# AwesomePeiweiPan/Droid-SLAM_Reserch

Measured on AMD Instinct MI355X. Metric: BA update iters/sec (2000-edge equivalents; 256 keyframes, 48x64), higher is better.
Workload: dtype f32; 1 GPU; 256-keyframe / 2000-edge global BA, 48x64, t0=1, lm=1e-5 ep=1e-2 (BASELINE configs[2]); edges_total=2000, solve=fp64 dense Cholesky on device, chol_failed=False

## Files before the change

droid-slam_reserch_amd/csrc/api.hip:

```cpp
#include <hip/hip_runtime.h>
#include <stdarg.h>
#include <stdio.h>

#include <map>
#include <mutex>

#include "../../include/droid_backends_hip.h"
#include "../../include/droid_test_hooks_hip.h"
#include "../../include/droid_heads_hip.h"
#include "../../include/droid_motion_encode_hip.h"
#include "../../include/droid_update_hip.h"
#include "ba_internal.hpp"
#include "graph.hpp"
#include "launchers.hpp"

using namespace droid;

static thread_local char g_err[512] = "";

static std::map<const void*, int*> g_mirror;
static std::mutex g_mirror_mu;
struct HintState { int* ptr; int tag; };
static std::map<const void*, HintState> g_hint;
static int g_hint_tag = 0;
// ... 241 lines not shown
static void enqueue_build(const BaView& v, const float* poses, const float* disps, const float* intrinsics,
                          const float* disps_sens, const float* targets, const float* weights, const float* eta,
                          const int64_t* ii, const int64_t* jj, bool motion_only, hipStream_t s, Between between) {
  const BaLaunchPlan plan = ba_launch_plan(v);
  for (int stage = 0; stage < 3; stage++) {
    launch_build_stage(v, plan, poses, disps, intrinsics, disps_sens, targets, weights, eta, ii, jj, motion_only, stage, s);
    between();
  }
}
template <class Between>
static void enqueue_solve_update(const BaView& v, float* poses, float* disps, const float* intrinsics, const float* weights,
                                 const int64_t* ii, const int64_t* jj, float lm, float ep, bool motion_only, float* dx_out,
                                 float* dz_out, int* status_mirror, hipStream_t s, Between between) {
  const CholSystem c(v);
  if (v.E <= 0) launch_chol_preset(c, s);
  const bool single = launch_chol_factor(c, (double)lm, (double)ep, s);
  between();
  launch_chol_backsolve(c, single, s);
  between();
  launch_update(v, poses, disps, intrinsics, weights, ii, jj, v.xsol, dx_out, dz_out, motion_only, s, status_mirror);
  between();
}

static int ba_build_impl(const float* poses, const float* disps, const float* intrinsics,
                         const float* disps_sens, const float* targets, const float* weights,
                         const float* eta, const int64_t* ii, const int64_t* jj, const BaDims& d, void* workspace,
                         size_t workspace_bytes, void* stream, int packed) {
  BaView v;
  int rc = ba_view(v, workspace, workspace_bytes, d);
  if (rc) return rc;
  v.packed = packed;
  hints_of(v, workspace, false);
  if (!poses || !disps || !intrinsics) return fail(DROID_E_ARG, "ba: null %s", "state pointer");
// ... 91 lines not shown
}

int droid_ba_solve_update_overlap(float* poses, float* disps, const float* intrinsics, const float* weights,
                                  const int64_t* ii, const int64_t* jj, int E, int nbuf, int H, int W, int M,
                                  int t0, int t1, int epoch, int motion_only, float* dx_out, float* dz_out,
                                  void* workspace, size_t workspace_bytes, void* stream) {
  BaView v;
  int rc = ba_view(v, workspace, workspace_bytes, BaDims{E, nbuf, H, W, M, t0, t1, motion_only});
  if (!rc) rc = solve_update_check(poses, disps, intrinsics, weights, ii, jj, E, motion_only);
  if (rc) return rc;
  if (E <= 0 || epoch <= 0) return fail(DROID_E_ARG, "ba_solve_update_overlap: needs %s", "edges (the build presets the solver scratch) and epoch > 0");
  hipStream_t s = (hipStream_t)stream;
  const CholSystem c(v);
  if (!launch_chol_factor_overlap(c, v.ov_ready, epoch, s))
    return fail(DROID_E_ARG, "ba_solve_update_overlap: %s", "the single-launch solver is not available for this system (unpack and call droid_ba_solve_update)");
  launch_chol_backsolve(c, true, s);
  launch_update(v, poses, disps, intrinsics, weights, ii, jj, v.xsol, dx_out, dz_out, motion_only != 0, s,
                mirror_of(workspace));
  return check_hip("ba_solve_update_overlap");
}

int droid_ba_solve_update(float* poses, float* disps, const float* intrinsics, const float* weights,
                          const int64_t* ii, const int64_t* jj, int E, int nbuf, int H, int W, int M,
                          int t0, int t1, float lm, float ep, int motion_only, float* dx_out,
                          float* dz_out, void* workspace, size_t workspace_bytes, void* stream) {
  BaView v;
  int rc = ba_view(v, workspace, workspace_bytes, BaDims{E, nbuf, H, W, M, t0, t1, motion_only});
  if (!rc) rc = solve_update_check(poses, disps, intrinsics, weights, ii, jj, E, motion_only);
  if (rc) return rc;
  enqueue_solve_update(v, poses, disps, intrinsics, weights, ii, jj, lm, ep, motion_only != 0, dx_out, dz_out,
                       mirror_of(workspace), (hipStream_t)stream, [] {});
// ... 555 lines not shown
```

droid-slam_reserch_amd/csrc/ba_internal.hpp:

```cpp
#pragma once
#include <hip/hip_runtime.h>
#include <stddef.h>
#include <stdint.h>

namespace droid {

constexpr int LIN_THREADS = 256;
constexpr int LIN_PPT = 2;
constexpr int LIN_CP = LIN_THREADS * LIN_PPT;
constexpr int LIN_WAVES = LIN_THREADS / 64;
constexpr int CHOL_NB = 64;
__host__ __device__ inline int chol_ld(int n) { return (n + 1 + 15) & ~15; }
__host__ __device__ inline size_t chol_flag_words(int n) { return 2 * ((size_t)(n + 1 + CHOL_NB - 1) / CHOL_NB) + 8; }
__host__ __device__ inline int chol_tile_index(int nrb, int bi, int bj) { return bj * nrb - bj * (bj - 1) / 2 + (bi - bj); }
__host__ __device__ inline size_t chol_tiles(int n) {
  const int nb = (n + CHOL_NB - 1) / CHOL_NB, nrb = (n + 1 + CHOL_NB - 1) / CHOL_NB;
  return (size_t)chol_tile_index(nrb, nb, nb);
}
__host__ __device__ inline size_t chol_mbuf_offset(int n) { return ((size_t)(n + CHOL_NB - 1) / CHOL_NB) * CHOL_NB * CHOL_NB; }
__host__ __device__ inline size_t chol_lfin_offset(int n) { return 2 * chol_mbuf_offset(n); }
__host__ __device__ inline size_t chol_ldiag_doubles(int n) { return chol_lfin_offset(n) + chol_tiles(n) * CHOL_NB * CHOL_NB; }
__host__ __device__ inline int chol_bs_pairs_grid(int nb) { return (nb + 1) / 2; }
__host__ __device__ inline int chol_bs_pairs_owner(int col) { return col / 2; }
__host__ __device__ inline int chol_bs_pairs_first(int wg) { return 2 * wg; }

__host__ __device__ inline size_t pk_colbase(int n, int J) {
  return (size_t)CHOL_NB * ((size_t)J * (size_t)(n + 1) - (size_t)CHOL_NB * (size_t)J * (size_t)(J - 1) / 2);
}
// ... 188 lines not shown
};

void launch_wave_reduce32_test(const float* in, float* out, hipStream_t s);
void launch_lin_test(const BaView& v, const float* poses, const float* disps, const float* intr, const float* sens,
                     const float* targets, const float* weights, const float* eta, const int64_t* ii, const int64_t* jj,
                     bool motion_only, bool ragged, hipStream_t s);
void launch_prep(const BaView& v, const int64_t* ii, const int64_t* jj, hipStream_t s);
void launch_unpack_system(const BaView& v, hipStream_t s);
void launch_build_stage(const BaView& v, const BaLaunchPlan& plan, const float* poses, const float* disps,
                        const float* intr, const float* sens, const float* targets, const float* weights,
                        const float* eta, const int64_t* ii, const int64_t* jj, bool motion_only,
                        int stage, hipStream_t s);
void launch_update(const BaView& v, float* poses, float* disps, const float* intr, const float* weights,
                   const int64_t* ii, const int64_t* jj, const double* x, float* dx_out, float* dz_out,
                   bool motion_only, hipStream_t s, int* status_mirror = nullptr);
void launch_chol_preset(const CholSystem& c, hipStream_t s);
bool launch_chol_factor(const CholSystem& c, double lm, double ep, hipStream_t s);
void launch_chol_backsolve(const CholSystem& c, bool factor_single, hipStream_t s);
void launch_chol_solve(const CholSystem& c, double lm, double ep, hipStream_t s, bool preset_done);

void launch_unpack_cols(const BaView& v, int J0, int J1, double lm, double ep, int epoch, hipStream_t s);
bool launch_chol_factor_overlap(const CholSystem& c, const int* ready, int epoch, hipStream_t s);
bool chol_overlap_available(int n);

}
```

droid-slam_reserch_amd/csrc/chol.hip:

```cpp
#include <hip/hip_runtime.h>
#include <mutex>

#include <cstdint>
#include <cstdlib>

#include "ba_internal.hpp"
#include "launchers.hpp"

namespace droid {

constexpr int NB = CHOL_NB;

#ifdef CHOL_STAMPS
__device__ unsigned long long g_chol_stamps[64 * 16];
__device__ unsigned long long g_bs_stamps[64 * 8];
__shared__ unsigned long long g_chol_lstamps[16];
extern "C" int droid_debug_chol_stamps(unsigned long long* out) {
  return (int)hipMemcpyFromSymbol(out, HIP_SYMBOL(g_chol_stamps), sizeof(unsigned long long) * 64 * 16);
}
extern "C" int droid_debug_bs_stamps(unsigned long long* out) {
  return (int)hipMemcpyFromSymbol(out, HIP_SYMBOL(g_bs_stamps), sizeof(unsigned long long) * 64 * 8);
}
#define STEP_STAMP(slot)                                                                                      \
  do { if (threadIdx.x == 0 && panel && (blockIdx.x < 2))                                                      \
// ... 1 lines not shown
#define LDS_STAMP(slot)                                                                                       \
  do { if (threadIdx.x == 0 && panel && (bi - kp < 2)) {                                                       \
    g_chol_lstamps[slot] = wall_clock64();                                                                    \
    if ((slot) == 2) { g_chol_lstamps[14] = 0; g_chol_lstamps[15] = 0; g_chol_lstamps[9] = 0; }               \
    if ((slot) == 8)                                                                                          \
      for (int ss = 0; ss < 16; ss++)                                                                         \
        if (ss < 11 || ss > 13) g_chol_stamps[((k + 1) & 31) * 32 + (bi - kp) * 16 + ss] = g_chol_lstamps[ss]; \
  } } while (0)
#define TILE_STAMP(slot) do { if (PERSIST) LDS_STAMP(slot); else STEP_STAMP(slot); } while (0)
#define GEMM_STAMP_AT(slot) do { if (ASSIGN && threadIdx.x == 0 && g_chol_lstamps[slot] == 0) g_chol_lstamps[slot] = wall_clock64(); } while (0)
#define GEMM_STAMP_ENTERED() GEMM_STAMP_AT(9)
#define GEMM_STAMP_OPERANDS() do { asm volatile("s_waitcnt vmcnt(0) lgkmcnt(0)" ::: "memory"); GEMM_STAMP_AT(14); } while (0)
#define GEMM_STAMP_DONE(acc) do { asm volatile("s_nop 15\n s_nop 15" : "+v"(acc)); GEMM_STAMP_AT(15); } while (0)
#define WAIT_STAMP(slot) do { if (t == 0 && panel && (bi - kp < 2)) g_chol_stamps[(kp & 31) * 32 + (bi - kp) * 16 + (slot)] = wall_clock64(); } while (0)
#define BS_STAMP(slot) do { if (threadIdx.x == 0 && blockIdx.x < 64) g_bs_stamps[blockIdx.x * 8 + (slot)] = wall_clock64(); } while (0)
#else
#define TILE_STAMP(slot) do { } while (0)
#define GEMM_STAMP_ENTERED() do { } while (0)
#define GEMM_STAMP_OPERANDS() do { } while (0)
#define GEMM_STAMP_DONE(acc) do { } while (0)
#define WAIT_STAMP(slot) do { } while (0)
#define BS_STAMP(slot) do { } while (0)
#endif
#ifdef OV_DEBUG
__device__ unsigned long long g_ov_dbg[64];
extern "C" int droid_debug_overlap_stamps(unsigned long long* out) {
  return (int)hipMemcpyFromSymbol(out, HIP_SYMBOL(g_ov_dbg), sizeof(unsigned long long) * 64);
}
#define OV_STAMP_ENTERED() do { if (blockIdx.x == 0 && threadIdx.x == 0) g_ov_dbg[63] = wall_clock64(); } while (0)
#define OV_STAMP_DIAG(bi, bj, k) do { if (threadIdx.x == 0 && (bi) == (bj) && (bj) == (k) + 1 && (bj) < 62) g_ov_dbg[bj] = wall_clock64(); } while (0)
#else
// ... 68 lines not shown
}

template <bool COH = false>
__device__ __forceinline__ void store_tile64(gbl_f64* __restrict__ S, const lds_f64* __restrict__ src,
                                             int ld, int r0, int c0, int row_begin, int row_end,
                                             int ncols, bool lower) {
  const int t = threadIdx.x & 255;
  if (COH) {
#pragma unroll
    for (int it = 0; it < 8; it++) {
      const int idx2 = it * 256 + t;
      const int i = idx2 >> 5, j = (idx2 & 31) * 2;
      if (r0 + i >= row_begin && r0 + i < row_end && j < ncols) {
        gbl_f64* p = &S[(size_t)(r0 + i) * ld + c0 + j];
        const f64x2 v = *(const lds_f64x2*)&src[i * LDP + j];
        if (j + 1 < ncols) asm volatile("global_store_dwordx4 %0, %1, off sc1" ::"v"(p), "v"(v) : "memory");
        else gstore<true>(p, v[0]);
      }
    }
    return;
  }
#pragma unroll
  for (int it = 0; it < 16; it++) {
    const int idx = it * 256 + t;
    const int i = idx >> 6, j = idx & 63;
    if (r0 + i >= row_begin && r0 + i < row_end && j < ncols && (!lower || j <= i))
      S[(size_t)(r0 + i) * ld + c0 + j] = src[i * LDP + j];
  }
}

__device__ __forceinline__ double readlane_f64(double v, int lane) {
// ... 52 lines not shown
  a[J] *= y;
  w[J] *= y;
  asm volatile("s_nop 1" : "+v"(a[J]));
#pragma unroll
  for (int c = J + 1; c < 16; c++) {
    switch (c) {
#define DROID_CASE(CC) case CC: if (CC > J) { fmac_bcast<J, CC>(a[CC], a[J], a[J]); fmac_bcast<J, CC>(w[CC], a[J], w[J]); } break;
      DROID_CASE(1) DROID_CASE(2) DROID_CASE(3) DROID_CASE(4) DROID_CASE(5) DROID_CASE(6) DROID_CASE(7) DROID_CASE(8)
      DROID_CASE(9) DROID_CASE(10) DROID_CASE(11) DROID_CASE(12) DROID_CASE(13) DROID_CASE(14) DROID_CASE(15)
#undef DROID_CASE
      default: break;
    }
  }
}

__device__ __forceinline__ void wave_potrf16(lds_f64* Lb, lds_f64* Wl, const lds_f64* Idn, int* fail, bool report) {
  const int lane = threadIdx.x & 63, row = lane & 15;
  __builtin_amdgcn_s_setprio(3);
  double a[16], w[16];
#pragma unroll
  for (int c = 0; c < 16; c++) {
    a[c] = Lb[row * LDP + c];
    w[c] = Idn[row * WLP + c];
  }
  double ylast = 0.0;
  potrf16_pivot<0>(a, w, ylast);   potrf16_pivot<1>(a, w, ylast);   potrf16_pivot<2>(a, w, ylast);
  potrf16_pivot<3>(a, w, ylast);   potrf16_pivot<4>(a, w, ylast);   potrf16_pivot<5>(a, w, ylast);
  potrf16_pivot<6>(a, w, ylast);   potrf16_pivot<7>(a, w, ylast);   potrf16_pivot<8>(a, w, ylast);
  potrf16_pivot<9>(a, w, ylast);   potrf16_pivot<10>(a, w, ylast);  potrf16_pivot<11>(a, w, ylast);
  potrf16_pivot<12>(a, w, ylast);  potrf16_pivot<13>(a, w, ylast);  potrf16_pivot<14>(a, w, ylast);
  potrf16_pivot<15>(a, w, ylast);
// ... 119 lines not shown
    if (++spins > CFP_SPIN_LIMIT || ((spins & 255) == 0 && cfp_load(abortf) == 1)) {
      cfp_report_stall(fail, abortf);
      break;
    }
    __builtin_amdgcn_s_sleep(1);
  }
#pragma unroll
  for (int it = 0; it < 2; it++) {
    const int u = it * 256 + t;
    const int i = u >> 3, j = 16 * sp + (u & 7) * 2;
    if (!ok[it]) v[it] = (f64x2){0.0, 0.0};
    *(lds_f64x2*)(&dst[i * LDP + j]) = v[it];
  }
}

__shared__ double g_cholB0[NB * LDP];
__shared__ double g_cholB1[NB * LDP];
__shared__ double g_cholB2[NB * LDP];
__shared__ double g_cholBT[NB * LDP];
__shared__ double g_cholWl[4 * WLB];
__shared__ double g_cholIdn[WLB];

__device__ __forceinline__ void chol_strip_out(gbl_f64* __restrict__ S, int ld, gbl_f64* __restrict__ slot,
                                                         const lds_f64* __restrict__ BT, int r0, int c0, int wk, int nrows,
                                                         int p, int* done_flag, int done_value) {
  const int lane = threadIdx.x & 63;
  const int rb = max(r0, c0 + wk) - r0, re = min(r0 + NB, nrows) - r0;
  const int i0 = lane >> 3, j = 16 * p + (lane & 7) * 2;
  auto uniform = [](const gbl_f64* q) {
    const unsigned long long a = (unsigned long long)q;
    const unsigned lo = __builtin_amdgcn_readfirstlane((unsigned)a), hi = __builtin_amdgcn_readfirstlane((unsigned)(a >> 32));
    return (const gbl_f64*)(((unsigned long long)hi << 32) | lo);
  };
  const gbl_f64* sbase = uniform(S + (size_t)r0 * ld + c0);
  const gbl_f64* sslot = uniform(slot);
  unsigned off_slot = (unsigned)((i0 * NB + j) * 8), off_mat = (unsigned)((i0 * ld + j) * 8);
// ... 20 lines not shown
    off_mat += step_mat;
  }
  if (done_flag != nullptr) {
    asm volatile("s_waitcnt vmcnt(0)" ::: "memory");
    if (lane == 0) cfp_store(done_flag, done_value);
  }
}

template <bool PERSIST, bool OV = false>
__device__ __forceinline__ void chol_tile(gbl_f64* __restrict__ S, int n, int ld, int k, int bi, int bj,
                                          int* __restrict__ fail, double lm, double ep,
                                          gbl_f64* __restrict__ Ldiag, int* __restrict__ done,
                                          int* __restrict__ abortf, bool coh_first_arg = false, int k_last_arg = -2) {
  const bool coh_first = OV && coh_first_arg;
  const int k_last = OV ? k_last_arg : -2;
  lds_f64* const B0 = DROID_LDS(g_cholB0);
  lds_f64* const B1 = DROID_LDS(g_cholB1);
  lds_f64* const B2 = DROID_LDS(g_cholB2);
  lds_f64* const BT = DROID_LDS(g_cholBT);
  lds_f64* const Wl = DROID_LDS(g_cholWl);
  lds_f64* const Idn = DROID_LDS(g_cholIdn);
  const int nrows = n + 1;
  const int kp = k + 1;
  if (bj > bi) return;
  const int t = threadIdx.x, wave = t >> 6, lane = t & 63;
  const int grp = wave >> 2, w4 = wave & 3;
  const int fr = lane & 15, fg = lane >> 4;
  const int r0 = bi * NB, q0 = bj * NB;
  const int c0 = kp * NB;
  const int wk = min(NB, n - c0);
  const bool panel = (bj == kp);
  const bool diag = panel && (bi == kp);
  f64x4 acc[4];

  if (!panel) {
    if (k < 0) {
// ... 228 lines not shown
        for (int i = 0; i < 4; i++) Cq[(fg + 4 * i) * LDP + fr] = acc[i];
        f64x4 m = {0.0, 0.0, 0.0, 0.0};
#pragma unroll
        for (int kk = 0; kk < 16; kk += 4)
          m = __builtin_amdgcn_mfma_f64_16x16x4f64(Cq[fr * LDP + kk + fg], Wl[WLB * q + (kk + fg) * WLP + fr], m, 0, 0, 0);
#pragma unroll
        for (int i = 0; i < 4; i++) Cq[(fg + 4 * i) * LDP + fr] = m[i];
      }
      gbl_f64* Mj = Ldiag + chol_mbuf_offset(n) + (size_t)kp * NB * NB;
#pragma unroll
      for (int it = 0; it < 8; it++) {
        const int u = it * 64 + lane;
        const int i = 16 * g + (u >> 5), j2 = (u & 31) * 2;
        f64x2 v = *(const lds_f64x2*)&BT[i * LDP + j2];
        if (r0 + i >= n) v = (f64x2){0.0, 0.0};
        *(gbl_f64x2*)&Mj[i * NB + j2] = v;
      }
    }
  }
  if (PERSIST && diag) {
#pragma unroll
    for (int e = t; e < 1024; e += 512) {
      const int pb = e >> 8, j = (e >> 4) & 15, kk = e & 15;
      const int br = pb == 3 ? 1 : 0, bc = pb == 3 ? 2 : pb + 1;
      B2[(16 * br + j) * LDP + 16 * bc + kk] = Wl[WLB * pb + WLP * j + kk];
    }
    __syncthreads();
  }
  if (grp == 0) {
    if (diag) {
      if (PERSIST) store_tile64(Ldiag + (size_t)kp * NB * NB, B2, NB, 0, 0, 0, NB, NB, false);
      else store_tile64(S, B2, ld, c0, c0, c0, c0 + wk, wk, true);
    }
  } else if (solve_rows && !PERSIST) {
    store_tile64(S, BT, ld, r0, c0, max(r0, c0 + wk), min(r0 + NB, nrows), wk, false);
  }
  if (!PERSIST) TILE_STAMP(9);
}

__global__ __launch_bounds__(512) void chol_step_kernel(double* __restrict__ S, int n, int ld, int k,
                                                        int* __restrict__ fail, double lm, double ep) {
  chol_tile<false>((gbl_f64*)S, n, ld, k, k + 1 + (int)blockIdx.x, k + 1 + (int)blockIdx.y, fail, lm, ep, nullptr,
                   nullptr, nullptr);
}


template <bool OV>
__device__ __attribute__((noinline)) void chol_tile_persist(double* __restrict__ S, int n, int ld, int k, int bi,
                                                            int bj, int* __restrict__ fail, double lm, double ep,
                                                            double* __restrict__ Ldiag, int* __restrict__ done,
// ... 12 lines not shown
  if (lane == 0 && flagged) in.flag = &done[bi];
  else if (lane == 1 && flagged && bj != bi) in.flag = &done[bj];
  else if (lane == 2 && k >= 0 && panel && bi != bj) { in.flag = &dver[bj]; in.need = k; }
  else if (OV && lane == 3 && k == cfp_first_step(bj)) { in.flag = &ready[bj]; in.need = epoch; }
  else if (OV && (lane == 4 || lane == 5) && k >= 0 && (panel || bj == k + 2))
    in.slot = lfin_slot((gbl_f64*)Ldiag, n, lane == 4 ? bi : bj, k);
  return in;
}

__device__ __forceinline__ void cfp_publish_diag(int* dver, int bj, int version) {
  asm volatile("s_waitcnt vmcnt(0)" ::: "memory");
  __syncthreads();
  if (threadIdx.x == 0) cfp_store(&dver[bj], version);
}

template <bool OV>
__global__ __launch_bounds__(512) void chol_factor_persistent_kernel(
    double* __restrict__ S, int n, int ld, int* __restrict__ fail, double lm, double ep, int* __restrict__ flags,
    double* __restrict__ Ldiag, const int* __restrict__ ready, int epoch);

template <>
__global__ __launch_bounds__(512) void chol_factor_persistent_kernel<false>(
    double* __restrict__ S, int n, int ld, int* __restrict__ fail, double lm, double ep, int* __restrict__ flags,
    double* __restrict__ Ldiag, const int* __restrict__, int) {
  __shared__ int s_abort;
  const int nb = (n + NB - 1) / NB;
  const int nrb = (n + 1 + NB - 1) / NB;
  int *done = flags, *dver = flags + nrb, *abortf = flags + 2 * nrb;
  const int G = (int)gridDim.x, wg = (int)blockIdx.x, t = (int)threadIdx.x;
  int total = 0;
  for (int j = 0; j < nb; j++) total += nrb - j;
  {
    int cs = 0;
    for (int j = 0; j < nb; j++) {
      if (j >= 1 && (cs % G) == wg) {
        const int i = j * NB + t;
        if (t < NB && i < n) {
          const double d = S[(size_t)i * ld + i];
          gstore<true>((gbl_f64*)&S[(size_t)i * ld + i], d + (ep + lm * d));
// ... 42 lines not shown
        }
        if (t == 0) {
          s_abort = ok ? 0 : 1;
          if (!ok) cfp_report_stall(fail, abortf);
        }
      }
      WAIT_STAMP(12);
      __syncthreads();
      if (s_abort) return;
      chol_tile_persist<false>(S, n, ld, k, bi, bj, fail, lm, ep, Ldiag, done, abortf, false, k);
      if (!panel && bi == bj) cfp_publish_diag(dver, bj, k + 1);
      WAIT_STAMP(13);
    }
    colstart += nrb - kp;
  }
}

template <>
__global__ __launch_bounds__(512) void chol_factor_persistent_kernel<true>(
    double* __restrict__ S, int n, int ld, int* __restrict__ fail, double lm, double ep, int* __restrict__ flags,
    double* __restrict__ Ldiag, const int* __restrict__ ready, int epoch) {
  constexpr int MAXT = 12;
  __shared__ int s_ti[MAXT], s_tj[MAXT], s_nx[MAXT], s_nt, s_pick, s_klast;
  const int nb = (n + NB - 1) / NB;
  const int nrb = (n + 1 + NB - 1) / NB;
  int *done = flags, *dver = flags + nrb, *abortf = flags + 2 * nrb;
  const int G = (int)gridDim.x, wg = (int)blockIdx.x, t = (int)threadIdx.x;
  const int total = (int)chol_tiles(n);
  {
    int cs = 0;
    for (int j = 0; j < nb; j++) {
      if (j >= 1 && (cs % G) == wg) cfp_publish_diag(dver, j, 0);
      cs += nrb - j;
    }
  }
  OV_STAMP_ENTERED();
// ... 278 lines not shown
    DROID_BS_BLOCK(1)
    DROID_BS_BLOCK(0)
#undef DROID_BS_BLOCK
#undef DROID_BS_WTERM
#undef DROID_BS_STEP
    BS_STAMP(2);
    if (FAST && j < nb - 1) xsol -= poll_matvec(j + 1, Mc);
    if (__double_as_longlong(xsol) == BSP_SENTINEL) xsol = __longlong_as_double(0x7ff8000000000000LL);
    BS_STAMP(4);
    if (t < wj) __hip_atomic_store(&x[c0 + t], xsol, __ATOMIC_RELAXED, __HIP_MEMORY_SCOPE_AGENT);
    BS_STAMP(5);
  }
}

#ifdef CHOL_STAMPS
#define BS_STAMP_W(slot, wv) do { if (threadIdx.x == 64 * (wv) && blockIdx.x < 64) g_bs_stamps[blockIdx.x * 8 + (slot)] = wall_clock64(); } while (0)
#else
#define BS_STAMP_W(slot, wv) do { } while (0)
#endif

struct BspTileRegs { f64x2 v[4]; };
__device__ __forceinline__ BspTileRegs bsp_tile_issue(const gbl_f64* __restrict__ src, size_t pitch, int rows_valid) {
  const int t = threadIdx.x;
  BspTileRegs r;
#pragma unroll
  for (int it = 0; it < 4; it++) {
    const int idx2 = it * 512 + t, i = idx2 >> 5, j = (idx2 & 31) * 2;
    const bool ok = i < rows_valid;
    r.v[it] = *(const gbl_f64x2*)(src + (ok ? (size_t)i * pitch + j : 0));
    if (!ok) r.v[it] = (f64x2){0.0, 0.0};
  }
  return r;
}
__device__ __forceinline__ void bsp_tile_store(lds_f64* __restrict__ dst, const BspTileRegs& r) {
  const int t = threadIdx.x;
#pragma unroll
  for (int it = 0; it < 4; it++) {
    const int idx2 = it * 512 + t, i = idx2 >> 5, j = (idx2 & 31) * 2;
    *(lds_f64x2*)(&dst[i * LDP + j]) = r.v[it];
  }
}

constexpr int BSP_DC = 10 * 256;
__device__ __forceinline__ int bsp_dc_source(int e) {
  const int blk = e >> 7, i = (e & 127) >> 3, j = (e & 7) * 2;
  int br, bc;
  if (blk < 6) {
    br = blk < 1 ? 1 : (blk < 3 ? 2 : 3);
    bc = blk - br * (br - 1) / 2;
  } else {
    br = blk == 9 ? 1 : 0;
    bc = blk == 9 ? 2 : blk - 5;
  }
  return (16 * br + i) * NB + 16 * bc + j;
}

__device__ __forceinline__ void bsp_times_inverse(lds_f64* T, const lds_f64* D, int g, int lane) {
  const int fr = lane & 15, fg = lane >> 4;
// ... 22 lines not shown

template <int NN>
__device__ __forceinline__ double bsp_dot(const double* col, const lds_f64* xs) {
  double a0 = 0.0, a1 = 0.0, a2 = 0.0, a3 = 0.0;
#pragma unroll
  for (int r = 0; r < NN; r += 4) {
    const f64x2 x01 = *(const lds_f64x2*)&xs[r], x23 = *(const lds_f64x2*)&xs[r + 2];
    a0 = fma(col[r + 0], x01[0], a0);
    a1 = fma(col[r + 1], x01[1], a1);
    a2 = fma(col[r + 2], x23[0], a2);
    a3 = fma(col[r + 3], x23[1], a3);
  }
  return (a0 + a1) + (a2 + a3);
}

__global__ __launch_bounds__(512) void chol_backsolve_pairs_kernel(
    double* __restrict__ S_, int n, int ld, double* __restrict__ x, int* __restrict__ err,
    const double* __restrict__ Ldiag_) {
  __shared__ double Dc[2][BSP_DC];
  __shared__ double Nt[3][NB * LDP];
  __shared__ double xs[8][NB];
  __shared__ double far_part[8][NB];
  __shared__ double near_part[8][NB];
  __shared__ double us[2][NB];
  __shared__ int dead;
  const gbl_f64* const S = (const gbl_f64*)S_;
  const gbl_f64* const Ldiag = (const gbl_f64*)Ldiag_;
  const int t = threadIdx.x, w = t >> 6, l = t & 63;
  const int nb = (n + NB - 1) / NB, G = gridDim.x, J = blockIdx.x;
  const int b = chol_bs_pairs_first(J), a = b + 1;
  const bool has_a = a < nb;
  const bool above = a + 1 < nb;
  const bool above2 = a + 2 < nb;
  const int ch = w & 1, rq = w >> 1;
  lds_f64* const xw = DROID_LDS(xs[w]);
  BS_STAMP_W(0, 0);
  if (t == 0) dead = 0;

  const int ra = (a + 1) * NB, rb = (a + 2) * NB;
  BspTileRegs t0, t1, t2;
  f64x2 dreg[5];
  if (above) {
    t1 = bsp_tile_issue(S + (size_t)ra * ld + (size_t)b * NB, ld, n - ra);
    if (above2) {
      t2 = bsp_tile_issue(S + (size_t)rb * ld + (size_t)b * NB, ld, n - rb);
      t0 = bsp_tile_issue(S + (size_t)rb * ld + (size_t)a * NB, ld, n - rb);
    }
#pragma unroll
    for (int it = 0; it < 5; it++) {
      const int idx2 = it * 512 + t, which = idx2 >= BSP_DC / 2 ? 1 : 0;
      dreg[it] = *(const gbl_f64x2*)(Ldiag + (size_t)(b + which) * NB * NB + bsp_dc_source(idx2 - which * (BSP_DC / 2)));
    }
// ... 39 lines not shown
      bsp_times_inverse(DROID_LDS(Nt[1]), DROID_LDS(Dc[0]), w, l);
      if (above2) bsp_times_inverse(DROID_LDS(Nt[0]), DROID_LDS(Dc[1]), w, l);
    } else if (above2) {
      bsp_times_inverse(DROID_LDS(Nt[2]), DROID_LDS(Dc[0]), w - 4, l);
    }
  }
  BS_STAMP_W(1, 0);

  auto poll = [&](int gi, int lanes) -> double {
    double xv = 0.0;
    if (l < lanes && gi + l < n) {
      int spins = 0;
      while (true) {
        xv = __hip_atomic_load(&x[gi + l], __ATOMIC_RELAXED, __HIP_MEMORY_SCOPE_AGENT);
        if (__double_as_longlong(xv) != BSP_SENTINEL) break;
        if (++spins > (1 << 22)) {
          *(volatile int*)&dead = 1;
          atomicMax(err, 2);
          xv = 0.0;
          break;
        }
        __builtin_amdgcn_s_sleep(1);
      }
    }
    return xv;
  };

  double far = 0.0;
  for (int P = G - 1; P >= J + 2; P--) {
    if (*(volatile int*)&dead) break;
    const int r0 = 2 * P * NB + 32 * rq;
    const gbl_f64* col = S + (size_t)(b + ch) * NB + l;
    double Tc[32];
#pragma unroll
    for (int r = 0; r < 32; r++) {
      const int row = r0 + r;
      Tc[r] = col[(size_t)(row < n ? row : n - 1) * ld];
      if (row >= n) Tc[r] = 0.0;
    }
    const double xv = poll(r0, 32);
    if (l < 32) xw[l] = xv;
    far += bsp_dot<32>(Tc, xw);
  }
  DROID_LDS(far_part[w])[l] = far;
  BS_STAMP_W(2, 0);
  __syncthreads();
  if (dead) return;

  if (w == 4 || (w == 5 && has_a)) {
    const int c = w - 4;
    z -= (far_part[c][l] + far_part[2 + c][l]) + (far_part[4 + c][l] + far_part[6 + c][l]);
    const int rowb = l >> 4;
    double xsol = 0.0;
#define DROID_BSP_WTERM(ACC, C)                                                                         \
    asm volatile("v_fmac_f64_dpp %0, %1, %2 row_newbcast:" #C " row_mask:0xf bank_mask:0xf"             \
                 : "+v"(ACC) : "v"(z), "v"(keep[C]));
#define DROID_BSP_BLOCK(B)                                                                              \
    if (rowb == B) {                                                                                   \
      double xw0 = 0.0, xw1 = 0.0;                                                                     \
      asm volatile("s_nop 1" : "+v"(z));                                                               \
      DROID_BSP_WTERM(xw0, 0) DROID_BSP_WTERM(xw1, 1) DROID_BSP_WTERM(xw0, 2) DROID_BSP_WTERM(xw1, 3)  \
      DROID_BSP_WTERM(xw0, 4) DROID_BSP_WTERM(xw1, 5) DROID_BSP_WTERM(xw0, 6) DROID_BSP_WTERM(xw1, 7)  \
// ... 27 lines not shown
    if (ch == 1 && rq < 2) {
#pragma unroll
      for (int r = 0; r < 32; r++) Nc[r] = keep[r];
    } else {
      const lds_f64* T = DROID_LDS(ch == 1 ? Nt[0] : (rq < 2 ? Nt[1] : Nt[2])) + (32 * (rq & 1)) * LDP + l;
#pragma unroll
      for (int r = 0; r < 32; r++) Nc[r] = T[r * LDP];
    }
    const double xv = poll((a + 1) * NB + 32 * rq, 32);
    BS_STAMP_W(4, 0);
    if (l < 32) xw[l] = xv;
    near = bsp_dot<32>(Nc, xw);
  }
  DROID_LDS(near_part[w])[l] = near;
  __syncthreads();
  if (dead) return;
  BS_STAMP_W(5, 6);
  if (w == 6 || (w == 7 && has_a)) {
    const auto publish = [&](int c0, double v) {
      if (__double_as_longlong(v) == BSP_SENTINEL) v = __longlong_as_double(0x7ff8000000000000LL);
      if (c0 + l < n) __hip_atomic_store(&x[c0 + l], v, __ATOMIC_RELAXED, __HIP_MEMORY_SCOPE_AGENT);
    };
    double xb = us[0][l] - ((near_part[0][l] + near_part[2][l]) + (near_part[4][l] + near_part[6][l]));
    if (has_a) {
      const double xa = us[1][l] - ((near_part[1][l] + near_part[3][l]) + (near_part[5][l] + near_part[7][l]));
      if (w == 7) {
        publish(a * NB, xa);
        return;
      }
      xw[l] = (a * NB + l < n) ? xa : 0.0;
      xb -= bsp_dot<NB>(keep, xw);
    }
    BS_STAMP_W(6, 6);
    publish(b * NB, xb);
    BS_STAMP_W(7, 6);
  }
}

struct CholSwitches {
  bool multi_launch;
  bool cooperative;
  bool force_bs_refusal;
  int grid;
  int overlap_reserve;
  bool bs_pairs;
};
static const CholSwitches& chol_switches() {
  const auto is_set = [](const char* name) { return getenv(name) != nullptr; };
  const auto number = [](const char* name, int unset) { const char* v = getenv(name); return v ? atoi(v) : unset; };
  static const CholSwitches sw = {is_set("DROID_CHOL_MULTI_LAUNCH"), number("DROID_CHOL_COOPERATIVE", 0) != 0,
                                  is_set("DROID_CHOL_FORCE_BS_REFUSAL"), number("DROID_CHOL_GRID", 0),
                                  number("DROID_OVERLAP_RESERVE_CUS", 32), number("DROID_CHOL_BS_PAIRS", 1) != 0};
  return sw;
}

struct PersistState {
  hipStream_t last = nullptr;
  hipEvent_t ev = nullptr;
  bool any = false;
  int resident = -1;
};
static PersistState g_persist[64];
static std::mutex g_persist_mu;

static int chol_resident_workgroups() {
  int dev = 0;
  if (hipGetDevice(&dev) != hipSuccess || dev < 0 || dev >= 64) return 0;
// ... 34 lines not shown
  }
  if (!refuse && hipLaunchCooperativeKernel(fn, dim3(workgroups), dim3(threads), args, 0, s) == hipSuccess) return true;
  (void)hipGetLastError();
  return false;
}

__global__ __launch_bounds__(256) void chol_ldiag_to_sys_kernel(double* __restrict__ S, int n, int ld,
                                                                const double* __restrict__ Ldiag) {
  const int j = blockIdx.x, c0 = j * NB, wk = min(NB, n - c0);
  for (int idx = threadIdx.x; idx < NB * NB; idx += blockDim.x) {
    const int i = idx / NB, c = idx % NB;
    if (i < wk && c <= i) S[(size_t)(c0 + i) * ld + c0 + c] = Ldiag[(size_t)j * NB * NB + idx];
  }
}

static bool launch_factor_grid(const void* fn, CholSystem c, double lm, double ep, const int* ready, int epoch, int cap,
                               hipStream_t s) {
  void* args[] = {&c.S, &c.n, &c.ld, &c.fail, &lm, &ep, &c.flags, &c.ldiag, &ready, &epoch};
  return launch_spinning_grid(fn, chol_tiles(c.n) < (size_t)cap ? (int)chol_tiles(c.n) : cap, 512, args, s);
}

static int chol_overlap_cap(int n) {
  const CholSwitches& sw = chol_switches();
  const int nb = (n + NB - 1) / NB;
  if (n <= 0 || sw.cooperative || sw.multi_launch || nb < 2) return 0;
  const int resident = chol_resident_workgroups();
  if (resident < 8 || chol_tiles(n) > (size_t)10 * resident) return 0;
  const int cap = resident - (sw.overlap_reserve > 0 ? sw.overlap_reserve : 0);
  return (cap >= 8 && chol_tiles(n) <= (size_t)10 * cap) ? cap : 0;
}
bool chol_overlap_available(int n) { return chol_overlap_cap(n) > 0; }

bool launch_chol_factor_overlap(const CholSystem& c, const int* ready, int epoch, hipStream_t s) {
  if (!ready || (c.ld % 16) != 0 || (reinterpret_cast<uintptr_t>(c.S) % 128) != 0) return false;
  const int cap = chol_overlap_cap(c.n);
  if (cap == 0) return false;
  return launch_factor_grid((const void*)chol_factor_persistent_kernel<true>, c, 0.0, 0.0, ready, epoch, cap, s);
}

bool launch_chol_factor(const CholSystem& c, double lm, double ep, hipStream_t s) {
  if (c.n <= 0) return false;
  if (int cap = chol_single_launch(c)) {
    const int grid = chol_switches().grid;
    if (grid >= 8 && grid < cap) cap = grid;
    if (launch_factor_grid((const void*)chol_factor_persistent_kernel<false>, c, lm, ep, nullptr, 0, cap, s)) return true;
  }
  const int nb = (c.n + NB - 1) / NB;
  const int nrb = (c.n + 1 + NB - 1) / NB;
  for (int k = -1; k + 1 < nb; k++)
    hipLaunchKernelGGL(chol_step_kernel, dim3(nrb - k - 1, k < 0 ? 2 : nb - k - 1), dim3(512), 0, s, c.S, c.n,
                       c.ld, k, c.fail, lm, ep);
  return false;
}

extern "C" int droid_debug_bs_pairs_map(int nb, int* owner) {
  for (int j = 0; j < nb; j++) owner[j] = chol_bs_pairs_owner(j);
  return chol_bs_pairs_grid(nb);
}

void launch_chol_backsolve(const CholSystem& c, bool factor_single, hipStream_t s) {
  const int nb = (c.n + NB - 1) / NB;
  if (nb >= 2 && nb <= BSP_MAX_BLOCKS) {
    CholSystem a = c;
    const double* ld_arg = factor_single ? c.ldiag : nullptr;
    void* args[] = {&a.S, &a.n, &a.ld, &a.x, &a.fail, &ld_arg};
    const bool pairs = factor_single && chol_switches().bs_pairs;
    const void* fn = pairs ? (const void*)chol_backsolve_pairs_kernel
                   : factor_single ? (const void*)chol_backsolve_persistent_kernel<true>
                                   : (const void*)chol_backsolve_persistent_kernel<false>;
    if (launch_spinning_grid(fn, pairs ? chol_bs_pairs_grid(nb) : nb, pairs ? 512 : 256, args, s,
                             chol_switches().force_bs_refusal)) return;
  }
  if (factor_single)
    hipLaunchKernelGGL(chol_ldiag_to_sys_kernel, dim3(nb), dim3(256), 0, s, c.S, c.n, c.ld, c.ldiag);
  for (int k = nb - 1; k >= 0; k--) {
    const int c0 = k * NB;
    hipLaunchKernelGGL(chol_backsolve_kernel, dim3(1 + (c0 + 255) / 256), dim3(256), 0, s, c.S, c.n,
                       c.ld, k, c.x);
  }
}

void launch_chol_preset(const CholSystem& c, hipStream_t s) {
  (void)hipMemsetAsync(c.fail, 0, sizeof(int), s);
  const size_t xbytes = sizeof(double) * (size_t)c.n, fbytes = sizeof(int) * chol_flag_words(c.n);
  const char* xb = reinterpret_cast<const char*>(c.x);
  const char* fb = reinterpret_cast<const char*>(c.flags);
  if (fb >= xb + xbytes && fb - xb <= (ptrdiff_t)(xbytes + 4096)) {
    (void)hipMemsetAsync(c.x, 0xFF, (size_t)(fb - xb) + fbytes, s);
  } else {
    (void)hipMemsetAsync(c.x, 0xFF, xbytes, s);
    (void)hipMemsetAsync(c.flags, 0xFF, fbytes, s);
  }
  (void)hipMemsetAsync(c.ldiag + chol_lfin_offset(c.n), 0xFF, sizeof(double) * chol_tiles(c.n) * NB * NB, s);
}

void launch_chol_solve(const CholSystem& c, double lm, double ep, hipStream_t s, bool preset_done) {
  if (c.n <= 0) return;
  if (!preset_done) launch_chol_preset(c, s);
  const bool single = launch_chol_factor(c, lm, ep, s);
  launch_chol_backsolve(c, single, s);
}

size_t CholSystem::scratch_doubles(int n) {
  if (n <= 0) return 0;
  return (size_t)(n + 1) * chol_ld(n) + chol_ldiag_doubles(n) + (chol_flag_words(n) + 1) / 2 + 16;
}
CholSystem::CholSystem(double* scratch, int n_, double* x_, int* fail_)
    : S(scratch), n(n_), ld(chol_ld(n_)), x(x_), fail(fail_) {
  ldiag = S + (size_t)(n + 1) * ld;
  flags = reinterpret_cast<int*>(ldiag + chol_ldiag_doubles(n));
}

__global__ void chol_pack_kernel(const double* __restrict__ A, const double* __restrict__ b,
                                 double* __restrict__ S, int n, int ld) {
  const size_t idx = (size_t)blockIdx.x * blockDim.x + threadIdx.x;
// ... 16 lines not shown
```

Baseline: 2084 iters/s.

## Fuse pairs backsolve into tail of persistent Cholesky factor kernel

The persistent factor kernel now runs the pairs backsolve in its trailing workgroups once they finish factoring. Each backsolve workgroup spin-waits on new per-block publication flags (Ldiag tile and M panel written) instead of waiting for a separate kernel launch. This removes one launch plus the kernel boundary, and lets the backsolve of late blocks overlap the end of the factorization. In exchange it moves the LDS into one shared buffer, doubles the flag words, adds store ordering nops, and adds more spin-wait stall risk.

```diff
diff --git a/droid-slam_reserch_amd/csrc/api.hip b/droid-slam_reserch_amd/csrc/api.hip
--- a/droid-slam_reserch_amd/csrc/api.hip
+++ b/droid-slam_reserch_amd/csrc/api.hip
@@ -279,9 +279,9 @@
                                  float* dz_out, int* status_mirror, hipStream_t s, Between between) {
   const CholSystem c(v);
   if (v.E <= 0) launch_chol_preset(c, s);
-  const bool single = launch_chol_factor(c, (double)lm, (double)ep, s);
+  const CholFactorRan ran = launch_chol_factor(c, (double)lm, (double)ep, s);
   between();
-  launch_chol_backsolve(c, single, s);
+  launch_chol_backsolve(c, ran, s);
   between();
   launch_update(v, poses, disps, intrinsics, weights, ii, jj, v.xsol, dx_out, dz_out, motion_only, s, status_mirror);
   between();
@@ -403,7 +403,7 @@
   const CholSystem c(v);
   if (!launch_chol_factor_overlap(c, v.ov_ready, epoch, s))
     return fail(DROID_E_ARG, "ba_solve_update_overlap: %s", "the single-launch solver is not available for this system (unpack and call droid_ba_solve_update)");
-  launch_chol_backsolve(c, true, s);
+  launch_chol_backsolve(c, CHOL_FACTOR_SINGLE, s);
   launch_update(v, poses, disps, intrinsics, weights, ii, jj, v.xsol, dx_out, dz_out, motion_only != 0, s,
                 mirror_of(workspace));
   return check_hip("ba_solve_update_overlap");
diff --git a/droid-slam_reserch_amd/csrc/ba_internal.hpp b/droid-slam_reserch_amd/csrc/ba_internal.hpp
--- a/droid-slam_reserch_amd/csrc/ba_internal.hpp
+++ b/droid-slam_reserch_amd/csrc/ba_internal.hpp
@@ -11,7 +11,8 @@
 constexpr int LIN_WAVES = LIN_THREADS / 64;
 constexpr int CHOL_NB = 64;
 __host__ __device__ inline int chol_ld(int n) { return (n + 1 + 15) & ~15; }
-__host__ __device__ inline size_t chol_flag_words(int n) { return 2 * ((size_t)(n + 1 + CHOL_NB - 1) / CHOL_NB) + 8; }
+__host__ __device__ inline size_t chol_pub_flag_offset(int n) { return 2 * ((size_t)(n + 1 + CHOL_NB - 1) / CHOL_NB) + 8; }
+__host__ __device__ inline size_t chol_flag_words(int n) { return 4 * ((size_t)(n + 1 + CHOL_NB - 1) / CHOL_NB) + 8; }
 __host__ __device__ inline int chol_tile_index(int nrb, int bi, int bj) { return bj * nrb - bj * (bj - 1) / 2 + (bi - bj); }
 __host__ __device__ inline size_t chol_tiles(int n) {
   const int nb = (n + CHOL_NB - 1) / CHOL_NB, nrb = (n + 1 + CHOL_NB - 1) / CHOL_NB;
@@ -230,9 +231,10 @@
 void launch_update(const BaView& v, float* poses, float* disps, const float* intr, const float* weights,
                    const int64_t* ii, const int64_t* jj, const double* x, float* dx_out, float* dz_out,
                    bool motion_only, hipStream_t s, int* status_mirror = nullptr);
+enum CholFactorRan { CHOL_FACTOR_STEPS = 0, CHOL_FACTOR_SINGLE = 1, CHOL_FACTOR_SINGLE_TAIL = 2 };
 void launch_chol_preset(const CholSystem& c, hipStream_t s);
-bool launch_chol_factor(const CholSystem& c, double lm, double ep, hipStream_t s);
-void launch_chol_backsolve(const CholSystem& c, bool factor_single, hipStream_t s);
+CholFactorRan launch_chol_factor(const CholSystem& c, double lm, double ep, hipStream_t s);
+void launch_chol_backsolve(const CholSystem& c, CholFactorRan factor, hipStream_t s);
 void launch_chol_solve(const CholSystem& c, double lm, double ep, hipStream_t s, bool preset_done);
 
 void launch_unpack_cols(const BaView& v, int J0, int J1, double lm, double ep, int epoch, hipStream_t s);
diff --git a/droid-slam_reserch_amd/csrc/chol.hip b/droid-slam_reserch_amd/csrc/chol.hip
--- a/droid-slam_reserch_amd/csrc/chol.hip
+++ b/droid-slam_reserch_amd/csrc/chol.hip
@@ -1,4 +1,5 @@
 #include <hip/hip_runtime.h>
+#include <atomic>
 #include <mutex>
 
 #include <cstdint>
@@ -39,7 +40,15 @@
 #define GEMM_STAMP_DONE(acc) do { asm volatile("s_nop 15\n s_nop 15" : "+v"(acc)); GEMM_STAMP_AT(15); } while (0)
 #define WAIT_STAMP(slot) do { if (t == 0 && panel && (bi - kp < 2)) g_chol_stamps[(kp & 31) * 32 + (bi - kp) * 16 + (slot)] = wall_clock64(); } while (0)
 #define BS_STAMP(slot) do { if (threadIdx.x == 0 && blockIdx.x < 64) g_bs_stamps[blockIdx.x * 8 + (slot)] = wall_clock64(); } while (0)
+__device__ unsigned long long g_tail_stamp;
+extern "C" int droid_debug_tail_stamp(unsigned long long* out) {
+  const unsigned long long zero = 0;
+  const int rc = (int)hipMemcpyFromSymbol(out, HIP_SYMBOL(g_tail_stamp), sizeof(unsigned long long));
+  return rc ? rc : (int)hipMemcpyToSymbol(HIP_SYMBOL(g_tail_stamp), &zero, sizeof(unsigned long long));
+}
+#define TAIL_STAMP_LOOP_EXIT() do { if (threadIdx.x == 0) atomicMax(&g_tail_stamp, (unsigned long long)wall_clock64()); } while (0)
 #else
+#define TAIL_STAMP_LOOP_EXIT() do { } while (0)
 #define TILE_STAMP(slot) do { } while (0)
 #define GEMM_STAMP_ENTERED() do { } while (0)
 #define GEMM_STAMP_OPERANDS() do { } while (0)
@@ -138,7 +147,7 @@
       if (r0 + i >= row_begin && r0 + i < row_end && j < ncols) {
         gbl_f64* p = &S[(size_t)(r0 + i) * ld + c0 + j];
         const f64x2 v = *(const lds_f64x2*)&src[i * LDP + j];
-        if (j + 1 < ncols) asm volatile("global_store_dwordx4 %0, %1, off sc1" ::"v"(p), "v"(v) : "memory");
+        if (j + 1 < ncols) asm volatile("global_store_dwordx4 %0, %1, off sc1\n\ts_nop 1" ::"v"(p), "v"(v) : "memory");
         else gstore<true>(p, v[0]);
       }
     }
@@ -221,7 +230,8 @@
   }
 }
 
-__device__ __forceinline__ void wave_potrf16(lds_f64* Lb, lds_f64* Wl, const lds_f64* Idn, int* fail, bool report) {
+__device__ __forceinline__ void wave_potrf16(lds_f64* __restrict__ Lb, lds_f64* __restrict__ Wl,
+                                             const lds_f64* __restrict__ Idn, int* fail, bool report) {
   const int lane = threadIdx.x & 63, row = lane & 15;
   __builtin_amdgcn_s_setprio(3);
   double a[16], w[16];
@@ -371,12 +381,15 @@
   }
 }
 
-__shared__ double g_cholB0[NB * LDP];
-__shared__ double g_cholB1[NB * LDP];
-__shared__ double g_cholB2[NB * LDP];
-__shared__ double g_cholBT[NB * LDP];
-__shared__ double g_cholWl[4 * WLB];
-__shared__ double g_cholIdn[WLB];
+constexpr int CHOL_LDS_B0 = 0, CHOL_LDS_B1 = NB * LDP, CHOL_LDS_B2 = 2 * NB * LDP, CHOL_LDS_BT = 3 * NB * LDP;
+constexpr int CHOL_LDS_WL = 4 * NB * LDP, CHOL_LDS_IDN = CHOL_LDS_WL + 4 * WLB;
+constexpr int CHOL_LDS_DOUBLES = CHOL_LDS_IDN + WLB;
+constexpr int BSP_DC = 10 * 256;
+constexpr int BSP_LDS_NT = 0, BSP_LDS_DC = 3 * NB * LDP, BSP_LDS_XS = BSP_LDS_DC + 2 * BSP_DC;
+constexpr int BSP_LDS_FAR = BSP_LDS_XS + 8 * NB, BSP_LDS_NEAR = BSP_LDS_FAR + 8 * NB, BSP_LDS_US = BSP_LDS_NEAR + 8 * NB;
+constexpr int BSP_LDS_DEAD = BSP_LDS_US + 2 * NB, BSP_LDS_DOUBLES = BSP_LDS_DEAD + 1;
+__shared__ double g_cholLds[CHOL_LDS_DOUBLES > BSP_LDS_DOUBLES ? CHOL_LDS_DOUBLES : BSP_LDS_DOUBLES];
+static_assert(sizeof(g_cholLds) + 64 <= 160 * 1024, "one workgroup per CU: 160 KB of LDS");
 
 __device__ __forceinline__ void chol_strip_out(gbl_f64* __restrict__ S, int ld, gbl_f64* __restrict__ slot,
                                                          const lds_f64* __restrict__ BT, int r0, int c0, int wk, int nrows,
@@ -427,12 +440,12 @@
                                           int* __restrict__ abortf, bool coh_first_arg = false, int k_last_arg = -2) {
   const bool coh_first = OV && coh_first_arg;
   const int k_last = OV ? k_last_arg : -2;
-  lds_f64* const B0 = DROID_LDS(g_cholB0);
-  lds_f64* const B1 = DROID_LDS(g_cholB1);
-  lds_f64* const B2 = DROID_LDS(g_cholB2);
-  lds_f64* const BT = DROID_LDS(g_cholBT);
-  lds_f64* const Wl = DROID_LDS(g_cholWl);
-  lds_f64* const Idn = DROID_LDS(g_cholIdn);
+  lds_f64* const B0 = DROID_LDS(g_cholLds) + CHOL_LDS_B0;
+  lds_f64* const B1 = DROID_LDS(g_cholLds) + CHOL_LDS_B1;
+  lds_f64* const B2 = DROID_LDS(g_cholLds) + CHOL_LDS_B2;
+  lds_f64* const BT = DROID_LDS(g_cholLds) + CHOL_LDS_BT;
+  lds_f64* const Wl = DROID_LDS(g_cholLds) + CHOL_LDS_WL;
+  lds_f64* const Idn = DROID_LDS(g_cholLds) + CHOL_LDS_IDN;
   const int nrows = n + 1;
   const int kp = k + 1;
   if (bj > bi) return;
@@ -691,7 +704,7 @@
         const int i = 16 * g + (u >> 5), j2 = (u & 31) * 2;
         f64x2 v = *(const lds_f64x2*)&BT[i * LDP + j2];
         if (r0 + i >= n) v = (f64x2){0.0, 0.0};
-        *(gbl_f64x2*)&Mj[i * NB + j2] = v;
+        asm volatile("global_store_dwordx4 %0, %1, off sc1\n\ts_nop 1" ::"v"(&Mj[i * NB + j2]), "v"(v) : "memory");
       }
     }
   }
@@ -706,11 +719,17 @@
   }
   if (grp == 0) {
     if (diag) {
-      if (PERSIST) store_tile64(Ldiag + (size_t)kp * NB * NB, B2, NB, 0, 0, 0, NB, NB, false);
+      if (PERSIST) store_tile64<true>(Ldiag + (size_t)kp * NB * NB, B2, NB, 0, 0, 0, NB, NB, false);
       else store_tile64(S, B2, ld, c0, c0, c0, c0 + wk, wk, true);
     }
   } else if (solve_rows && !PERSIST) {
     store_tile64(S, BT, ld, r0, c0, max(r0, c0 + wk), min(r0 + NB, nrows), wk, false);
+  }
+  if (PERSIST && (diag || (bi == kp + 1 && kp + 1 < (n + NB - 1) / NB))) {
+    int* there = done + chol_pub_flag_offset(n) + (diag ? 0 : (n + 1 + NB - 1) / NB) + kp;
+    asm volatile("s_waitcnt vmcnt(0)" ::: "memory");
+    __syncthreads();
+    if (t == 0) cfp_store(there, 1);
   }
   if (!PERSIST) TILE_STAMP(9);
 }
@@ -753,15 +772,20 @@
   if (threadIdx.x == 0) cfp_store(&dver[bj], version);
 }
 
+__device__ __attribute__((noinline)) void chol_bs_pairs_body(const double* __restrict__ S_, int n, int ld,
+                                                             double* __restrict__ x, int* __restrict__ err,
+                                                             const double* __restrict__ Ldiag_, int J, int G,
+                                                             int* __restrict__ flags);
+
 template <bool OV>
 __global__ __launch_bounds__(512) void chol_factor_persistent_kernel(
     double* __restrict__ S, int n, int ld, int* __restrict__ fail, double lm, double ep, int* __restrict__ flags,
-    double* __restrict__ Ldiag, const int* __restrict__ ready, int epoch);
+    double* __restrict__ Ldiag, const int* __restrict__ ready, int epoch, double* __restrict__ x);
 
 template <>
 __global__ __launch_bounds__(512) void chol_factor_persistent_kernel<false>(
     double* __restrict__ S, int n, int ld, int* __restrict__ fail, double lm, double ep, int* __restrict__ flags,
-    double* __restrict__ Ldiag, const int* __restrict__, int) {
+    double* __restrict__ Ldiag, const int* __restrict__, int, double* __restrict__ x) {
   __shared__ int s_abort;
   const int nb = (n + NB - 1) / NB;
   const int nrb = (n + 1 + NB - 1) / NB;
@@ -834,12 +858,18 @@
     }
     colstart += nrb - kp;
   }
+  TAIL_STAMP_LOOP_EXIT();
+  const int role = G - 1 - wg, roles = chol_bs_pairs_grid(nb);
+  if (x != nullptr && role < roles) {
+    __syncthreads();
+    chol_bs_pairs_body(S, n, ld, x, fail, Ldiag, role, roles, flags);
+  }
 }
 
 template <>
 __global__ __launch_bounds__(512) void chol_factor_persistent_kernel<true>(
     double* __restrict__ S, int n, int ld, int* __restrict__ fail, double lm, double ep, int* __restrict__ flags,
-    double* __restrict__ Ldiag, const int* __restrict__ ready, int epoch) {
+    double* __restrict__ Ldiag, const int* __restrict__ ready, int epoch, double* __restrict__) {
   constexpr int MAXT = 12;
   __shared__ int s_ti[MAXT], s_tj[MAXT], s_nx[MAXT], s_nt, s_pick, s_klast;
   const int nb = (n + NB - 1) / NB;
@@ -1148,7 +1178,7 @@
 }
 
 #ifdef CHOL_STAMPS
-#define BS_STAMP_W(slot, wv) do { if (threadIdx.x == 64 * (wv) && blockIdx.x < 64) g_bs_stamps[blockIdx.x * 8 + (slot)] = wall_clock64(); } while (0)
+#define BS_STAMP_W(slot, wv) do { if (threadIdx.x == 64 * (wv) && J < 64) g_bs_stamps[J * 8 + (slot)] = wall_clock64(); } while (0)
 #else
 #define BS_STAMP_W(slot, wv) do { } while (0)
 #endif
@@ -1175,7 +1205,6 @@
   }
 }
 
-constexpr int BSP_DC = 10 * 256;
 __device__ __forceinline__ int bsp_dc_source(int e) {
   const int blk = e >> 7, i = (e & 127) >> 3, j = (e & 7) * 2;
   int br, bc;
@@ -1228,20 +1257,26 @@
   return (a0 + a1) + (a2 + a3);
 }
 
-__global__ __launch_bounds__(512) void chol_backsolve_pairs_kernel(
-    double* __restrict__ S_, int n, int ld, double* __restrict__ x, int* __restrict__ err,
-    const double* __restrict__ Ldiag_) {
-  __shared__ double Dc[2][BSP_DC];
-  __shared__ double Nt[3][NB * LDP];
-  __shared__ double xs[8][NB];
-  __shared__ double far_part[8][NB];
-  __shared__ double near_part[8][NB];
-  __shared__ double us[2][NB];
-  __shared__ int dead;
+typedef lds_f64 lds_bsp_dc[BSP_DC];
+typedef lds_f64 lds_bsp_tile[NB * LDP];
+typedef lds_f64 lds_bsp_vec[NB];
+typedef __attribute__((address_space(3))) int lds_i32;
+__device__ __attribute__((noinline)) void chol_bs_pairs_body(const double* __restrict__ S_, int n, int ld,
+                                                             double* __restrict__ x, int* __restrict__ err,
+                                                             const double* __restrict__ Ldiag_, int J, int G,
+                                                             int* __restrict__ flags) {
+  lds_f64* const lds = DROID_LDS(g_cholLds);
+  lds_bsp_dc* const Dc = (lds_bsp_dc*)(lds + BSP_LDS_DC);
+  lds_bsp_tile* const Nt = (lds_bsp_tile*)(lds + BSP_LDS_NT);
+  lds_bsp_vec* const xs = (lds_bsp_vec*)(lds + BSP_LDS_XS);
+  lds_bsp_vec* const far_part = (lds_bsp_vec*)(lds + BSP_LDS_FAR);
+  lds_bsp_vec* const near_part = (lds_bsp_vec*)(lds + BSP_LDS_NEAR);
+  lds_bsp_vec* const us = (lds_bsp_vec*)(lds + BSP_LDS_US);
+  volatile lds_i32* const dead = (volatile lds_i32*)(lds + BSP_LDS_DEAD);
   const gbl_f64* const S = (const gbl_f64*)S_;
   const gbl_f64* const Ldiag = (const gbl_f64*)Ldiag_;
   const int t = threadIdx.x, w = t >> 6, l = t & 63;
-  const int nb = (n + NB - 1) / NB, G = gridDim.x, J = blockIdx.x;
+  const int nb = (n + NB - 1) / NB;
   const int b = chol_bs_pairs_first(J), a = b + 1;
   const bool has_a = a < nb;
   const bool above = a + 1 < nb;
@@ -1249,7 +1284,39 @@
   const int ch = w & 1, rq = w >> 1;
   lds_f64* const xw = DROID_LDS(xs[w]);
   BS_STAMP_W(0, 0);
-  if (t == 0) dead = 0;
+  if (t == 0) *dead = 0;
+  int* const abortf = flags ? flags + 2 * ((n + 1 + NB - 1) / NB) : nullptr;
+  if (flags != nullptr) {
+    if (w == 0) {
+      const int nrb = (n + 1 + NB - 1) / NB, top = has_a ? a : b, need = 4 * top + 3;
+      const int *done = flags, *ldiag_there = flags + chol_pub_flag_offset(n), *m_there = ldiag_there + nrb;
+      bool ok = true;
+      int spins = 0;
+      while (true) {
+        bool sat = true;
+        for (int r = top + 1 + l; r < nrb; r += 64) sat = sat && cfp_load(&done[r]) >= need;
+        if (l == 0) sat = sat && cfp_load(&ldiag_there[b]) >= 1;
+        if (l == 1 && has_a) sat = sat && cfp_load(&ldiag_there[a]) >= 1;
+        if (l == 2 && has_a) sat = sat && cfp_load(&m_there[b]) >= 1;
+        if (l == 3 && above) sat = sat && cfp_load(&m_there[a]) >= 1;
+        if (l == 4 && top + 1 == nrb) sat = sat && cfp_load(&done[top]) >= need;
+        if (__all(sat)) break;
+        spins++;
+        if (spins > CFP_SPIN_LIMIT || ((spins & 255) == 0 && __any(cfp_load(abortf) == 1))) {
+          ok = false;
+          break;
+        }
+        __builtin_amdgcn_s_sleep(1);
+      }
+      if (l == 0 && !ok) {
+        *dead = 1;
+        cfp_report_stall(err, abortf);
+      }
+    }
+    __syncthreads();
+    if (*dead) return;
+    __builtin_amdgcn_fence(__ATOMIC_ACQUIRE, "agent");
+  }
 
   const int ra = (a + 1) * NB, rb = (a + 2) * NB;
   BspTileRegs t0, t1, t2;
@@ -1319,8 +1386,8 @@
       while (true) {
         xv = __hip_atomic_load(&x[gi + l], __ATOMIC_RELAXED, __HIP_MEMORY_SCOPE_AGENT);
         if (__double_as_longlong(xv) != BSP_SENTINEL) break;
-        if (++spins > (1 << 22)) {
-          *(volatile int*)&dead = 1;
+        if (++spins > (1 << 22) || (abortf != nullptr && (spins & 255) == 0 && cfp_load(abortf) == 1)) {
+          *dead = 1;
           atomicMax(err, 2);
           xv = 0.0;
           break;
@@ -1333,7 +1400,7 @@
 
   double far = 0.0;
   for (int P = G - 1; P >= J + 2; P--) {
-    if (*(volatile int*)&dead) break;
+    if (*dead) break;
     const int r0 = 2 * P * NB + 32 * rq;
     const gbl_f64* col = S + (size_t)(b + ch) * NB + l;
     double Tc[32];
@@ -1350,7 +1417,7 @@
   DROID_LDS(far_part[w])[l] = far;
   BS_STAMP_W(2, 0);
   __syncthreads();
-  if (dead) return;
+  if (*dead) return;
 
   if (w == 4 || (w == 5 && has_a)) {
     const int c = w - 4;
@@ -1408,7 +1475,7 @@
   }
   DROID_LDS(near_part[w])[l] = near;
   __syncthreads();
-  if (dead) return;
+  if (*dead) return;
   BS_STAMP_W(5, 6);
   if (w == 6 || (w == 7 && has_a)) {
     const auto publish = [&](int c0, double v) {
@@ -1431,6 +1498,12 @@
   }
 }
 
+__global__ __launch_bounds__(512) void chol_backsolve_pairs_kernel(
+    double* __restrict__ S, int n, int ld, double* __restrict__ x, int* __restrict__ err,
+    const double* __restrict__ Ldiag) {
+  chol_bs_pairs_body(S, n, ld, x, err, Ldiag, (int)blockIdx.x, (int)gridDim.x, nullptr);
+}
+
 struct CholSwitches {
   bool multi_launch;
   bool cooperative;
@@ -1438,13 +1511,15 @@
   int grid;
   int overlap_reserve;
   bool bs_pairs;
+  bool bs_tail;
 };
 static const CholSwitches& chol_switches() {
   const auto is_set = [](const char* name) { return getenv(name) != nullptr; };
   const auto number = [](const char* name, int unset) { const char* v = getenv(name); return v ? atoi(v) : unset; };
   static const CholSwitches sw = {is_set("DROID_CHOL_MULTI_LAUNCH"), number("DROID_CHOL_COOPERATIVE", 0) != 0,
                                   is_set("DROID_CHOL_FORCE_BS_REFUSAL"), number("DROID_CHOL_GRID", 0),
-                                  number("DROID_OVERLAP_RESERVE_CUS", 32), number("DROID_CHOL_BS_PAIRS", 1) != 0};
+                                  number("DROID_OVERLAP_RESERVE_CUS", 32), number("DROID_CHOL_BS_PAIRS", 1) != 0,
+                                  number("DROID_CHOL_BS_TAIL", 1) != 0};
   return sw;
 }
 
@@ -1509,10 +1584,12 @@
   }
 }
 
+static int chol_factor_grid(int n, int cap) { return chol_tiles(n) < (size_t)cap ? (int)chol_tiles(n) : cap; }
 static bool launch_factor_grid(const void* fn, CholSystem c, double lm, double ep, const int* ready, int epoch, int cap,
-                               hipStream_t s) {
-  void* args[] = {&c.S, &c.n, &c.ld, &c.fail, &lm, &ep, &c.flags, &c.ldiag, &ready, &epoch};
-  return launch_spinning_grid(fn, chol_tiles(c.n) < (size_t)cap ? (int)chol_tiles(c.n) : cap, 512, args, s);
+                               bool tail, hipStream_t s) {
+  double* x = tail ? c.x : nullptr;
+  void* args[] = {&c.S, &c.n, &c.ld, &c.fail, &lm, &ep, &c.flags, &c.ldiag, &ready, &epoch, &x};
+  return launch_spinning_grid(fn, chol_factor_grid(c.n, cap), 512, args, s);
 }
 
 static int chol_overlap_cap(int n) {
@@ -1530,22 +1607,32 @@
   if (!ready || (c.ld % 16) != 0 || (reinterpret_cast<uintptr_t>(c.S) % 128) != 0) return false;
   const int cap = chol_overlap_cap(c.n);
   if (cap == 0) return false;
-  return launch_factor_grid((const void*)chol_factor_persistent_kernel<true>, c, 0.0, 0.0, ready, epoch, cap, s);
-}
-
-bool launch_chol_factor(const CholSystem& c, double lm, double ep, hipStream_t s) {
-  if (c.n <= 0) return false;
+  return launch_factor_grid((const void*)chol_factor_persistent_kernel<true>, c, 0.0, 0.0, ready, epoch, cap, false, s);
+}
+
+static std::atomic<int> g_chol_path{0};
+extern "C" int droid_debug_chol_path() { return g_chol_path.load(); }
+
+CholFactorRan launch_chol_factor(const CholSystem& c, double lm, double ep, hipStream_t s) {
+  g_chol_path = CHOL_FACTOR_STEPS;
+  if (c.n <= 0) return CHOL_FACTOR_STEPS;
   if (int cap = chol_single_launch(c)) {
-    const int grid = chol_switches().grid;
-    if (grid >= 8 && grid < cap) cap = grid;
-    if (launch_factor_grid((const void*)chol_factor_persistent_kernel<false>, c, lm, ep, nullptr, 0, cap, s)) return true;
+    const CholSwitches& sw = chol_switches();
+    if (sw.grid >= 8 && sw.grid < cap) cap = sw.grid;
+    const int nb = (c.n + NB - 1) / NB;
+    const bool tail = sw.bs_tail && sw.bs_pairs && !sw.force_bs_refusal && nb <= BSP_MAX_BLOCKS &&
+                      chol_bs_pairs_grid(nb) <= chol_factor_grid(c.n, cap);
+    if (launch_factor_grid((const void*)chol_factor_persistent_kernel<false>, c, lm, ep, nullptr, 0, cap, tail, s)) {
+      g_chol_path = tail ? CHOL_FACTOR_SINGLE_TAIL : CHOL_FACTOR_SINGLE;
+      return tail ? CHOL_FACTOR_SINGLE_TAIL : CHOL_FACTOR_SINGLE;
+    }
   }
   const int nb = (c.n + NB - 1) / NB;
   const int nrb = (c.n + 1 + NB - 1) / NB;
   for (int k = -1; k + 1 < nb; k++)
     hipLaunchKernelGGL(chol_step_kernel, dim3(nrb - k - 1, k < 0 ? 2 : nb - k - 1), dim3(512), 0, s, c.S, c.n,
                        c.ld, k, c.fail, lm, ep);
-  return false;
+  return CHOL_FACTOR_STEPS;
 }
 
 extern "C" int droid_debug_bs_pairs_map(int nb, int* owner) {
@@ -1553,7 +1640,9 @@
   return chol_bs_pairs_grid(nb);
 }
 
-void launch_chol_backsolve(const CholSystem& c, bool factor_single, hipStream_t s) {
+void launch_chol_backsolve(const CholSystem& c, CholFactorRan factor, hipStream_t s) {
+  if (factor == CHOL_FACTOR_SINGLE_TAIL) return;
+  const bool factor_single = factor == CHOL_FACTOR_SINGLE;
   const int nb = (c.n + NB - 1) / NB;
   if (nb >= 2 && nb <= BSP_MAX_BLOCKS) {
     CholSystem a = c;
@@ -1564,8 +1653,12 @@
                    : factor_single ? (const void*)chol_backsolve_persistent_kernel<true>
                                    : (const void*)chol_backsolve_persistent_kernel<false>;
     if (launch_spinning_grid(fn, pairs ? chol_bs_pairs_grid(nb) : nb, pairs ? 512 : 256, args, s,
-                             chol_switches().force_bs_refusal)) return;
-  }
+                             chol_switches().force_bs_refusal)) {
+      g_chol_path = g_chol_path.load() % 10 + (pairs ? 10 : 20);
+      return;
+    }
+  }
+  g_chol_path = g_chol_path.load() % 10 + 30;
   if (factor_single)
     hipLaunchKernelGGL(chol_ldiag_to_sys_kernel, dim3(nb), dim3(256), 0, s, c.S, c.n, c.ld, c.ldiag);
   for (int k = nb - 1; k >= 0; k--) {
@@ -1592,8 +1685,7 @@
 void launch_chol_solve(const CholSystem& c, double lm, double ep, hipStream_t s, bool preset_done) {
   if (c.n <= 0) return;
   if (!preset_done) launch_chol_preset(c, s);
-  const bool single = launch_chol_factor(c, lm, ep, s);
-  launch_chol_backsolve(c, single, s);
+  launch_chol_backsolve(c, launch_chol_factor(c, lm, ep, s), s);
 }
 
 size_t CholSystem::scratch_doubles(int n) {
```

New measurement: 2081 iters/s. Within noise of the previous version (-0.2%).
